# deepreinforce-ai/CUDA-L2

Measured on AMD Instinct MI355X. Metric: HGEMM TFLOP/s, higher is better.
Workload: dtype f16

## Files before the change

cuda-l2_amd/build.py:

```python
from __future__ import annotations

import concurrent.futures as cf
import hashlib
import os
import shutil
import subprocess
import sys
from pathlib import Path

PKG_DIR = Path(__file__).resolve().parent
REPO_DIR = PKG_DIR.parent
CSRC = PKG_DIR / "csrc"
INCLUDE = REPO_DIR / "include"
BUILD = PKG_DIR / "build"
OBJ = BUILD / "obj"
_SUFFIX = os.environ.get("HGEMM_LIB_SUFFIX", "")
LIB_DIR = PKG_DIR / ("lib_" + _SUFFIX if _SUFFIX else "lib")
BIN_DIR = PKG_DIR / "bin"
ROCM = Path(os.environ.get("ROCM_PATH", "/opt/rocm"))
HIPCC = str(ROCM / "bin" / "hipcc")
ARCH = "gfx950"

LIB_SOURCES = [
    "hgemm_inst_g0.hip",
    "hgemm_inst_g1.hip",
    "hgemm_inst_g2.hip",
    "hgemm_inst_g3.hip",
    "hgemm_inst_g4.hip",
    "hgemm_registry.hip",
    "hgemm_plan.hip",
    "hgemm_api.hip",
    "hgemm_baselines.hip",
]

HIP_FLAGS = os.environ.get("HGEMM_EXTRA_HIPFLAGS", "").split() + [f"--offload-arch={ARCH}", "-O3", "-std=c++17", "-fPIC", "-Wall", "-Wno-unused-function",
             "-Wno-unused-result", "-Wno-unused-value", "-DROCBLAS_NO_DEPRECATED_WARNINGS", "-D__HIP_PLATFORM_AMD__"]


def _headers_digest() -> str:
    h = hashlib.sha256()
    for d in (CSRC, INCLUDE):
        for p in sorted(d.rglob("*")):
            if p.suffix in (".hpp", ".h", ".def", ".inc"):
                h.update(p.name.encode())
                h.update(p.read_bytes())
    return h.hexdigest()


def _run(cmd: list[str], verbose: bool) -> None:
    if verbose:
        print(" ".join(cmd), flush=True)
    res = subprocess.run(cmd, capture_output=True, text=True)
    if res.returncode != 0:
        sys.stderr.write(res.stdout + res.stderr)
        raise RuntimeError(f"build step failed ({res.returncode}): {' '.join(cmd)}")
    if verbose and (res.stdout or res.stderr):
        print(res.stdout + res.stderr, flush=True)


def compile_object(src: Path, extra_flags: list[str], hdr_digest: str, verbose: bool = False) -> Path:
    OBJ.mkdir(parents=True, exist_ok=True)
# ... 111 lines not shown
```

cuda-l2_amd/csrc/hgemm_api.hip:

```cpp
#include "hgemm_plan.hpp"
#include "../../include/hgemm_mi355x.h"

#include <algorithm>
#include <atomic>
#include <cmath>
#include <cstdint>
#include <cstdlib>
#include <cstring>
#include <mutex>
#include <vector>

using namespace hgemm_mi355x;

namespace {

thread_local int g_last_hip_error = 0;
#ifdef HGEMM_ABLATION
int g_debug_flags = 0;
#endif
#ifdef HGEMM_TIMELINE
unsigned long long* g_timeline = nullptr;
int g_timeline_slots = 0;
unsigned g_timeline_count = 0;
constexpr int kTimelineWgs = 1024;
// ... 182 lines not shown
        t.tail_first = (int)full; t.tail_tiles = (int)tail; t.splits = S; t.k_chunk = per_t * e.kgran;
        t.items = (int)tail * S;
        g.items = (int)full; set_raster_div(g); set_raster_div(t);
        p.form = FORM_HYBRID; p.slab_bytes = (size_t)t.items * e.bm * e.bn * sizeof(float);
        add(THUNK_ENTRY, g, std::min<long>(full, G), EPI_C16);
        add(THUNK_ENTRY, t, std::min<long>(t.items, G), EPI_SLAB);
        add(THUNK_TAIL_REDUCE, t, 0, EPI_SLAB);
        return p;
      }
    }
  }
  long launch_grid = (e.persistent_wgs > 0) ? std::min<long>(grid, e.persistent_wgs) : grid;
  if (epi == EPI_FUSED && e.persistent_wgs > kCUs && 2L * (e.lds_bytes + 64) > 160L * 1024) launch_grid = std::min<long>(launch_grid, kCUs);
  set_raster_div(g);
  add(THUNK_ENTRY, g, launch_grid, epi);
  if (epi == EPI_SLAB) add(THUNK_SPLITK_REDUCE, g, 0, EPI_SLAB);
  return p;
}

struct AltRow { int M, N, K; const char* cfg; int splits, group_m; };
const AltRow g_alt_rows[] = {
#include "hgemm_tuned_alternates.inc"
    {0, 0, 0, nullptr, 0, 0}};
struct PlanTriple { int cfg, splits, group_m; };
struct InsituChoice { int dev, M, N, K; PlanTriple plan; };
std::mutex g_insitu_mutex;
std::vector<InsituChoice> g_insitu;
std::atomic<unsigned> g_insitu_epoch{1};
std::atomic<int> g_insitu_mode{-1};
constexpr int kInsituReps = 5;
struct InsituMemo { unsigned epoch; int dev, M, N, K; PlanTriple plan; };
thread_local InsituMemo t_insitu_memo[32] = {};

bool insitu_enabled() {
  int mode = g_insitu_mode.load(std::memory_order_relaxed);
  if (mode < 0) {
    const char* e = getenv("HGEMM_MI355X_INSITU");
    int expected = -1;
    g_insitu_mode.compare_exchange_strong(expected, (e && *e && *e != '0') ? 1 : 0);
    mode = g_insitu_mode.load(std::memory_order_relaxed);
  }
  return mode == 1;
}

int insitu_candidates(int M, int N, int K, PlanTriple out[3]) {
  int n = 0;
  PlanTriple p0;
  if (hgemm_mi355x_plan(M, N, K, &p0.cfg, &p0.splits, &p0.group_m) != HGEMM_OK) return 0;
  out[n++] = p0;
  auto add = [&](PlanTriple p) {
    if (n >= 3 || p.cfg < 0 || p.cfg >= g_num_kernels || !k_ok(g_kernel_table[p.cfg], K)) return;
    for (int i = 0; i < n; ++i)
      if (out[i].cfg == p.cfg && out[i].splits == p.splits && out[i].group_m == p.group_m) return;
    out[n++] = p;
  };
  for (const AltRow* r = g_alt_rows; r->cfg; ++r)
    if (r->M == M && r->N == N && r->K == K) add({hgemm_mi355x_config_by_name(r->cfg), r->splits, r->group_m});
  std::call_once(g_tuned_once, build_tuned_index);
  if (p0.cfg >= 0 && !find_tuned(M, N, K) && K % 8 == 0 && (N & 3) == 0) {
    RankedPlan ranked[8];
    int nr = 0, c0, s0, g0;
    if (neighbour_plan(M, N, K, &c0, &s0, &g0, ranked, &nr)) {
      std::sort(ranked, ranked + nr, [](const RankedPlan& a, const RankedPlan& b) { return a.us < b.us; });
      for (int i = 0; i < nr; ++i) add({ranked[i].cfg, ranked[i].splits, ranked[i].group_m});
    }
  }
// ... 259 lines not shown
    return resolve_launch(config_id, splits_arg, group_m, b != nullptr, b_col_major != nullptr, aligned, M, N, K, lda, ldb, ldc, ruled_out);
  };
  LaunchPlan p = resolve();
  float* slabs = nullptr; unsigned* counters = nullptr;
  while (p.status == HGEMM_OK && p.slab_bytes) {
    const int st = ensure_workspace(p.slab_bytes, s, &slabs, &counters);
    if (st == HGEMM_OK) break;
    if (st != HGEMM_ERR_NO_WORKSPACE_INTERNAL && p.form != FORM_HYBRID) return st;
    ruled_out |= 1u << p.form;
    p = resolve();
  }
  if (p.status != HGEMM_OK) return p.status;
  for (int i = 0; i < p.n; ++i) {
    GemmArgs& g = p.d[i].g;
    g.A = (const f16*)a; g.Bt = (const f16*)b_col_major; g.C = (f16*)c;
    if (p.d[i].epi != EPI_C16) {
      g.partial = slabs;
      if (p.counters) g.counters = counters;
    }
    const TimingSlot ts = timing_slot(p.d[i].start, p.d[i].stop);
    switch (p.d[i].thunk) {
      case THUNK_ENTRY: g_kernel_table[config_id].launch(g, p.d[i].grid, s, p.d[i].epi, ts); break;
      case THUNK_SPLITK_REDUCE: launch_splitk_reduce(g.partial, g.C, M, N, ldc, g.splits, s, ts); break;
      case THUNK_TAIL_REDUCE: launch_tail_reduce(g, g_kernel_table[config_id].bm, g_kernel_table[config_id].bn, s, ts); break;
      case THUNK_RAGGED: launch_ragged(g, s, ts); break;
      case THUNK_GENERIC: launch_generic((const f16*)a, (const f16*)b, (f16*)c, M, N, K, lda, N, ldc, s, ts); break;
    }
  }
  hipError_t err = hipGetLastError();
  if (err != hipSuccess) { g_last_hip_error = (int)err; return HGEMM_ERR_HIP; }
  return HGEMM_OK;
}

int hgemm_mi355x_set_insitu(int enable) {
  const int old = insitu_enabled() ? 1 : 0;
  g_insitu_mode.store(enable ? 1 : 0);
  if (!enable) {
    std::lock_guard<std::mutex> lk(g_insitu_mutex);
    g_insitu.clear();
    g_insitu_epoch.fetch_add(1, std::memory_order_release);
  }
  return old;
}

int hgemm_mi355x_insitu_enabled(void) { return insitu_enabled() ? 1 : 0; }

int hgemm_mi355x_insitu_candidates(int M, int N, int K, int config_id[3], int splits[3], int group_m[3]) {
  if (M <= 0 || N <= 0 || K <= 0 || !config_id || !splits || !group_m) return 0;
  PlanTriple c[3];
  const int n = insitu_candidates(M, N, K, c);
  for (int i = 0; i < n; ++i) { config_id[i] = c[i].cfg; splits[i] = c[i].splits; group_m[i] = c[i].group_m; }
  return n;
}

int hgemm_mi355x_insitu_choice(int M, int N, int K, int* config_id, int* splits, int* group_m) {
  PlanTriple p;
  int dev = 0;
  if (hipGetDevice(&dev) != hipSuccess) { (void)hipGetLastError(); dev = 0; }
  if (!config_id || !splits || !group_m || !insitu_lookup(dev, M, N, K, &p)) return 0;
  *config_id = p.cfg; *splits = p.splits; *group_m = p.group_m;
  return 1;
}

int hgemm_mi355x_fp32(const void* a, const void* b, const void* bt, void* c, int M, int N, int K,
                      void* stream) {
  return run(HGEMM_ACC_FP32, a, b, bt, c, M, N, K, stream);
// ... 96 lines not shown
```

cuda-l2_amd/csrc/hgemm_inst.inc:

```
#include "hgemm_launch.hpp"

#define HGEMM_INST_0(...)
#define HGEMM_INST_1(...)
#define HGEMM_INST_2(...)
#define HGEMM_INST_3(...)
#define HGEMM_INST_4(...)
#if HGEMM_INST_GROUP == 0
#undef HGEMM_INST_0
#define HGEMM_INST_0(...) __VA_ARGS__
#elif HGEMM_INST_GROUP == 1
#undef HGEMM_INST_1
#define HGEMM_INST_1(...) __VA_ARGS__
#elif HGEMM_INST_GROUP == 2
#undef HGEMM_INST_2
#define HGEMM_INST_2(...) __VA_ARGS__
#elif HGEMM_INST_GROUP == 3
#undef HGEMM_INST_3
#define HGEMM_INST_3(...) __VA_ARGS__
#elif HGEMM_INST_GROUP == 4
#undef HGEMM_INST_4
#define HGEMM_INST_4(...) __VA_ARGS__
#else
#error "HGEMM_INST_GROUP must be 0..4"
#endif

namespace hgemm_mi355x {
#define HGEMM_THUNK(G, FN, ...) HGEMM_INST_##G(template void FN<__VA_ARGS__>(const GemmArgs&, int, hipStream_t, int, TimingSlot);)
#include "hgemm_thunks.inc"
}
```

cuda-l2_amd/csrc/hgemm_kernel.hpp:

```cpp
#pragma once

#include <hip/hip_runtime.h>
#include <stdint.h>
#include <type_traits>

namespace hgemm_mi355x {

using f16    = _Float16;
using f16x4  = __attribute__((ext_vector_type(4))) _Float16;
using f16x8  = __attribute__((ext_vector_type(8))) _Float16;
using f32x4  = __attribute__((ext_vector_type(4))) float;
using f32x16 = __attribute__((ext_vector_type(16))) float;

constexpr int BK        = 64;
constexpr int ROW_BYTES = BK * 2;
constexpr int NUM_XCD   = 8;

constexpr int ARG_NT_STORE      = 1;
constexpr int ARG_XCD_STAGGER   = 2;
constexpr int ARG_NT_LOADS      = 4;
constexpr int ARG_PHASE_OFFSET  = 8;
constexpr int ARG_WAVE_PRIORITY = 16;
constexpr int ARG_PHASE_OFFSET4 = 32;

// ... 149 lines not shown
}

template <int BYTES>
__device__ __forceinline__ void prefetch_kernargs() {
#if defined(__HIP_DEVICE_COMPILE__)
  const char* ka = (const char*)__builtin_amdgcn_kernarg_segment_ptr();
  unsigned d0, d1, d2, d3;
  if constexpr (BYTES > 192)
    asm volatile("s_load_dword %0, %4, 0x0\n\ts_load_dword %1, %4, 0x40\n\ts_load_dword %2, %4, 0x80\n\ts_load_dword %3, %4, 0xc0\n\ts_waitcnt lgkmcnt(0)"
                 : "=&s"(d0), "=&s"(d1), "=&s"(d2), "=&s"(d3) : "s"(ka));
  else if constexpr (BYTES > 128)
    asm volatile("s_load_dword %0, %3, 0x0\n\ts_load_dword %1, %3, 0x40\n\ts_load_dword %2, %3, 0x80\n\ts_waitcnt lgkmcnt(0)"
                 : "=&s"(d0), "=&s"(d1), "=&s"(d2) : "s"(ka));
  else if constexpr (BYTES > 64)
    asm volatile("s_load_dword %0, %2, 0x0\n\ts_load_dword %1, %2, 0x40\n\ts_waitcnt lgkmcnt(0)" : "=&s"(d0), "=&s"(d1) : "s"(ka));
  else
    asm volatile("s_load_dword %0, %1, 0x0\n\ts_waitcnt lgkmcnt(0)" : "=&s"(d0) : "s"(ka));
  (void)d0; (void)d1; (void)d2; (void)d3;
#endif
}

#ifdef HGEMM_ABLATION
#define HGEMM_DBG(g, bit) (((g).debug & (bit)) != 0)
#else
#define HGEMM_DBG(g, bit) false
#endif

constexpr int EPI_C16    = 0;
constexpr int EPI_SLAB   = 1;
constexpr int EPI_FUSED  = 2;
constexpr int EPI_STREAMK = 3;
constexpr int EPI_KTAIL = 8;
constexpr int EPI_KSTAGGER = 16;

template <int BM_, int BN_, int WM_, int WN_, int MI_, int NBUF_>
struct Cfg {
  static constexpr int BM = BM_, BN = BN_, WM = WM_, WN = WN_, MI = MI_, NBUF = NBUF_;
  static constexpr int NW          = WM * WN;
  static constexpr int THREADS     = NW * 64;
  static constexpr int TM          = BM / WM;
  static constexpr int TN          = BN / WN;
  static constexpr int FM          = TM / MI;
  static constexpr int FN          = TN / MI;
  static constexpr int STAGE_BYTES = (BM + BN) * ROW_BYTES;
  static constexpr int LDS_BYTES   = STAGE_BYTES * NBUF;
  static constexpr int NI_A        = BM / 8;
  static constexpr int NI          = (BM + BN) / 8;
  static constexpr int NJ          = (NI + NW - 1) / NW;
  static_assert(MI == 16 || MI == 32, "MFMA shape");
  static_assert(BM % (WM * MI) == 0 && BN % (WN * MI) == 0, "wave tile must be MFMA-aligned");
  static_assert(BM % 8 == 0 && BN % 8 == 0, "tile rows come in 8-row DMA pieces");
  static_assert(LDS_BYTES <= 160 * 1024, "LDS budget");
  static_assert(NBUF >= 2, "need at least double buffering");
  static_assert(NBUF == 2 || NI % NW == 0, "deep ring needs an even piece split");
};

template <int N>
__device__ __forceinline__ void wait_vmcnt() {
  asm volatile("s_waitcnt vmcnt(%0)" ::"n"(N) : "memory");
}

struct TileCoord {
  int split, m0, n0, k_begin, nk;
  int tile, item;
  float* slab;
  int slab_ld;
// ... 547 lines not shown
```

cuda-l2_amd/csrc/hgemm_kernel_sq.hpp:

```cpp
#pragma once

#include "hgemm_kernel_sp.hpp"

#ifndef HGEMM_SQ_SLACK
#define HGEMM_SQ_SLACK 6
#endif
#ifndef HGEMM_SQ_SLACK32
#define HGEMM_SQ_SLACK32 4
#endif
#ifndef HGEMM_SQ_RS64
#define HGEMM_SQ_RS64 2
#endif
#ifndef HGEMM_SQ_ABL
#define HGEMM_SQ_ABL 0
#endif

namespace hgemm_mi355x {

template <int BM_, int BN_, int WM_, int WN_, int KT_ = 1, int MI_ = 16>
struct CfgSQ : Cfg<BM_, BN_, WM_, WN_, MI_, 2> {
  using Base = Cfg<BM_, BN_, WM_, WN_, MI_, 2>;
  static constexpr int KT  = KT_;
  static constexpr int KS  = (MI_ == 16) ? 1 : 2;
  static constexpr int SL  = KT * KS;
  static constexpr int ACC = (MI_ == 16) ? 4 : 16;
  static constexpr int SUB_BYTES   = Base::STAGE_BYTES;
  static constexpr int STAGE_BYTES = KT * SUB_BYTES;
  static constexpr int LDS_BYTES   = 2 * STAGE_BYTES;
  static constexpr int NFA = Base::FM * SL, NFB = Base::FN * SL;
  static constexpr int T   = Base::FM * Base::FN * SL;
  static constexpr int PA  = Base::NI_A / Base::NW;
  static constexpr int PB  = Base::NJ - PA;
  static constexpr int NJA = KT * PA, NJB = KT * PB;
  static constexpr int RS  = (T >= 64) ? HGEMM_SQ_RS64 : 1;
  static constexpr int SLACK = (MI_ == 32) ? HGEMM_SQ_SLACK32 : (T >= 64) ? HGEMM_SQ_SLACK : (T >= 32 ? 6 : 2);
// ... 125 lines not shown
  constexpr int S = PHASE == 0 ? CFG::P : CFG::Q;
  const uint32_t lds_l = (uint32_t)(uintptr_t)(lds_void_t*)stage_l + (uint32_t)wave * 1024u;
  const uint32_t lds_e = (uint32_t)(uintptr_t)(lds_void_t*)stage_e + (uint32_t)wave * 1024u;
#pragma unroll
  for (int n = 0; n < T; ++n) {
    const int u = n / (FM * FN), i = (n / FN) % FM, j = n % FN;
    if (n == S) {
      __builtin_amdgcn_sched_barrier(0);
      if (!(HGEMM_SQ_ABL & 4)) __builtin_amdgcn_s_waitcnt(kWaitLgkm0);
      if (!(HGEMM_SQ_ABL & 1)) sp_sync();
    }
    sp_mfma_mi<CFG::MI>(i * FN + j, bf[u * FN + j], af[u * FM + i]);
    if (!(HGEMM_SQ_ABL & 16) && n % RS == 0 && n / RS < NLEAD) {
      const int r = n / RS;
      lead[r] = *(const f16x8*)((r / FLEAD ? lead1 : lead0) + (r % FLEAD) * CFG::MI * ROW_BYTES);
    }
    constexpr SqSlots<CFG, PHASE> tab{};
    const int l = (HGEMM_SQ_ABL & 8) ? -1 : tab.late[n], l1 = (HGEMM_SQ_ABL & 8) ? -1 : tab.late[n + 1];
    const int e = (HGEMM_SQ_ABL & 8) ? -1 : tab.early[n], e1 = (HGEMM_SQ_ABL & 8) ? -1 : tab.early[n + 1];
    const int r = (HGEMM_SQ_ABL & 16) ? -1 : tab.trail[n];
    if (l >= 0) { if constexpr (OP_L == 0) sq_piece_load<CFG, 0>(rs_l, voffA, D_L + l, kbyte_l); else sq_piece_load<CFG, 1>(rs_l, voffB, D_L + l, kbyte_l); }
    if (e >= 0) { if constexpr (OP_E == 0) sq_piece_load<CFG, 0>(rs_e, voffA, e, kbyte_e); else sq_piece_load<CFG, 1>(rs_e, voffB, e, kbyte_e); }
    if (r >= 0) trail[r] = *(const f16x8*)((r / FTRAIL ? trail1 : trail0) + (r % FTRAIL) * CFG::MI * ROW_BYTES);
    if (l1 >= 0) sq_piece_m0<CFG, OP_L>(lds_l, D_L + l1, l1 > 0);
    if (e1 >= 0) sq_piece_m0<CFG, OP_E>(lds_e, e1, e1 > 0);
    if (n == S - 2 && !(HGEMM_SQ_ABL & 2)) wait_vmcnt<CFG::NJA + CFG::NJB>();
    if (n == T - 3) {
      __builtin_amdgcn_sched_barrier(0);
      __builtin_amdgcn_s_waitcnt(kWaitLgkm0);
      __builtin_amdgcn_sched_barrier(0);
    }
  }
}
#endif

#define SQ_LOAD_ITEM(OP, ITEM)                                                                                 \
  do {                                                                                                         \
                                \
    if (nxt_item != (ITEM)) {                                                                                  \
      const TileCoord itc = map_logical(g, walk.base + walk.first + (ITEM) * walk.stride, BM, BN);             \
      nxt_item = (ITEM);                                                                                       \
      nxt_m0 = __builtin_amdgcn_readfirstlane(itc.m0); nxt_n0 = __builtin_amdgcn_readfirstlane(itc.n0);        \
      nxt_kb = __builtin_amdgcn_readfirstlane(itc.k_begin * 2);                                                \
             \
      nxt_nk = __builtin_amdgcn_readfirstlane(KTAIL ? sq_k_items(g, itc) / (BK * CFG::KT) : itc.nk / CFG::KT);           \
    }                                                                                                          \
    const uintptr_t addr = (OP) == 0 ? reinterpret_cast<uintptr_t>(g.A + (size_t)nxt_m0 * g.lda)               \
                                     : reinterpret_cast<uintptr_t>(g.Bt + (size_t)nxt_n0 * g.ldb);             \
    const uintptr_t uni = ((uintptr_t)(uint32_t)__builtin_amdgcn_readfirstlane((int)(addr >> 32)) << 32) |     \
                          (uint32_t)__builtin_amdgcn_readfirstlane((int)(uint32_t)addr);                       \
    const unsigned long long rows_ = (OP) == 0 ? (unsigned long long)(g.M - nxt_m0) : (unsigned long long)(g.N - nxt_n0); \
    const unsigned long long rem_ = rows_ * (unsigned long long)((OP) == 0 ? g.lda : g.ldb) * 2ull;            \
    const unsigned range_ = (unsigned)__builtin_amdgcn_readfirstlane((int)(rem_ > 0xFFFFFFFFull ? 0xFFFFFFFFu : (unsigned)rem_)); \
    if ((OP) == 0) rsA = __builtin_amdgcn_make_buffer_rsrc((void*)uni, 0, (int)range_, 0x00020000);            \
    else           rsB = __builtin_amdgcn_make_buffer_rsrc((void*)uni, 0, (int)range_, 0x00020000);            \
                                \
    const int stag_ = STAG ? (int)(((uint32_t)(blockIdx.x & (NUM_XCD - 1)) * (uint32_t)nxt_nk) >> 3) : 0;                   \
    cur[OP].kbyte0 = (uint32_t)nxt_kb; cur[OP].kwrap = nxt_nk - stag_;                                         \
    cur[OP].kbyte = (uint32_t)nxt_kb + (uint32_t)stag_ * (uint32_t)(CFG::KT * ROW_BYTES);                      \
    cur[OP].item = (ITEM); cur[OP].kt = 0; cur[OP].nk = nxt_nk;                                                \
  } while (0)

#define SQ_STEP_CURSOR(OP)                                                                   \
  do {                                                                                       \
    ++cur[OP].kt;                                                                            \
    cur[OP].kbyte += CFG::KT * ROW_BYTES;                                                    \
// ... 7 lines not shown
    } else if (cur[OP].item + 1 < walk.count) {               \
      SQ_LOAD_ITEM(OP, cur[OP].item + 1);                     \
    }                                                         \
  } while (0)

#define SQ_FRAG(STAGE, OPOFF, H, U) ((STAGE) + (CFG::KT == 2 ? (H) * CFG::SUB_BYTES : 0) + (OPOFF) + \
                                     foff[CFG::KT == 2 ? (U) : (H)][CFG::KT == 2 ? 0 : (U) % CFG::KS])
#define SQ_K_STEP(YS, ZS, ADV0, ADV1)                                                                           \
  do {                                                                                                          \
    char* st  = smem + (step & 1) * CFG::STAGE_BYTES;                                                           \
    char* nst = smem + ((step + 1) & 1) * CFG::STAGE_BYTES;                                                     \
    sq_interval<CFG, 0>(fX, fU, fV, SQ_FRAG(st, b_base_off, 1, 0), SQ_FRAG(st, b_base_off, 1, 1),               \
                        ZS, SQ_FRAG(nst, a_base_off, 1, 0), SQ_FRAG(nst, a_base_off, 1, 1), wave, voffA, voffB, \
                        rsA, st, cur[0].kbyte, rsB, st, cur[1].kbyte);                                          \
    ADV0;                                                                                                       \
    sq_interval<CFG, 1>(YS, fV, fX, SQ_FRAG(nst, a_base_off, 0, 0), SQ_FRAG(nst, a_base_off, 0, 1),             \
                        fU, SQ_FRAG(nst, b_base_off, 0, 0), SQ_FRAG(nst, b_base_off, 0, 1), wave, voffA, voffB, \
                        rsB, st, cur[1].kbyte, rsA, nst, cur[0].kbyte);                                         \
    ADV1;                                                                                                       \
    ++step;                                                                                                     \
  } while (0)

__device__ __forceinline__ int sq_k_items(const GemmArgs& g, const TileCoord& tc) {
  return (tc.split + 1 == g.splits ? g.K : tc.k_begin + g.k_chunk) - tc.k_begin;
}

template <class CFG, int EPI_>
__global__ void __launch_bounds__(CFG::THREADS) hgemm_tn_sq_kernel(const GemmArgs g) {
  prefetch_kernargs<sizeof(GemmArgs)>();
#if defined(__HIP_DEVICE_COMPILE__)
  constexpr int EPI = EPI_ & 7;
  constexpr bool KTAIL = (EPI_ & EPI_KTAIL) != 0;
  constexpr bool STAG = (EPI_ & EPI_KSTAGGER) != 0;
  static_assert(!KTAIL || CFG::MI == 16, "the K tail is built from 16x16x32 fragments");
  static_assert(!(KTAIL && STAG), "the kstagger variant takes whole stages only (the host drops the flag when K has a tail)");
  constexpr int BM = CFG::BM, BN = CFG::BN, FM = CFG::FM, FN = CFG::FN, NJ = CFG::NJ, MI = CFG::MI;
  constexpr int NFA = CFG::NFA, NFB = CFG::NFB;
  constexpr int NQ = CFG::ACC / 4;

  constexpr bool STAGED = EPI == SP_EPI_WIDE && CFG::WGS == 1 && sp_staged_ok<CFG>(CFG::LDS_BYTES);
#ifdef HGEMM_TIMELINE
  constexpr int TL_EXTRA = 64;
  constexpr int FLAG_BYTES = 64;
#else
  constexpr int TL_EXTRA = 0;
  constexpr int FLAG_BYTES = (CFG::WGS == 2 && EPI != SP_EPI_FUSED) ? 0 : 64;
#endif
  constexpr int STAGED_BYTES = STAGED ? CFG::NW * SP_STAGED_BYTES_PER_WAVE : 0;
  __shared__ __attribute__((aligned(1024))) char smem[CFG::LDS_BYTES + FLAG_BYTES + STAGED_BYTES + TL_EXTRA];

  const int tid  = threadIdx.x;
  HGEMM_TL_STAMP(smem + CFG::LDS_BYTES, 0, tid);
  HGEMM_TL_REALTIME(smem + CFG::LDS_BYTES, 1, tid);
  const int lane = tid & 63;
  const int wave = __builtin_amdgcn_readfirstlane(tid >> 6);
  const int wave_m = wave / CFG::WN;
  const int wave_n = wave % CFG::WN;

  const ItemWalk walk = persistent_walk(g.items);
  if (walk.count == 0) return;

  if (g.flags & (ARG_PHASE_OFFSET | ARG_PHASE_OFFSET4)) {
    const int j = (int)(blockIdx.x >> 3);
    constexpr int both = ARG_PHASE_OFFSET | ARG_PHASE_OFFSET4;
    const int groups = (g.flags & both) == both ? 8 : (g.flags & ARG_PHASE_OFFSET4) ? 4 : 2, grp = j & (groups - 1);
    if (grp != 0 && walk.count > 1) {
      const int nk0 = g.k_chunk / (BK * CFG::KT);
      const int period = nk0 * 2 * CFG::T * (CFG::MI == 32 ? 32 : 16) + CFG::BM * CFG::BN / 12;
      const int spacing = min(period / groups, CFG::BM * CFG::BN / 6);
#pragma clang loop unroll(disable)
      for (int c = 0; c < spacing * grp; c += 1024) __builtin_amdgcn_s_sleep(16);
    }
  }
  if constexpr (CFG::WGS == 2) {
    if (g.flags & ARG_WAVE_PRIORITY) {
      unsigned hw;
      asm volatile("s_getreg_b32 %0, hwreg(HW_REG_HW_ID)" : "=s"(hw));
      if (hw & 1u) __builtin_amdgcn_s_setprio(2);
    }
  }

// ... 37 lines not shown
    }
    SQ_ADVANCE(0);
    SQ_ADVANCE(1);
  }
  __builtin_amdgcn_sched_barrier(0);
#pragma unroll
  for (; zi < NZ; ++zi) sp_zero_acc(zi);
  HGEMM_TL_STAMP(smem + CFG::LDS_BYTES + 64 + STAGED_BYTES, 1, tid);
  wait_vmcnt<CFG::NJA + CFG::NJB>();
  __builtin_amdgcn_s_barrier();
  HGEMM_TL_STAMP(smem + CFG::LDS_BYTES + 64 + STAGED_BYTES, 2, tid);

  f16x8 fX[NFA], fY[NFA], fZ[NFA], fU[NFB], fV[NFB];
#pragma unroll
  for (int r = 0; r < NFA; ++r) {
    fX[r] = *(const f16x8*)(SQ_FRAG(smem, a_base_off, 0, r / FM) + (r % FM) * MI * ROW_BYTES);
    fY[r] = *(const f16x8*)(SQ_FRAG(smem, a_base_off, 1, r / FM) + (r % FM) * MI * ROW_BYTES);
  }
#pragma unroll
  for (int r = 0; r < NFB; ++r) fU[r] = *(const f16x8*)(SQ_FRAG(smem, b_base_off, 0, r / FN) + (r % FN) * MI * ROW_BYTES);
  __builtin_amdgcn_sched_barrier(0);
  __builtin_amdgcn_s_waitcnt(kWaitLgkm0);
  sp_sync();
#pragma unroll
  for (int p = 0; p < CFG::DA; ++p) sq_issue_piece<CFG, 0>(rsA, voffA, smem, wave, p, cur[0].kbyte);

  int step = 0;
  HGEMM_TL_STAMP(smem + CFG::LDS_BYTES, 2, tid);
#pragma clang loop unroll(disable)
  for (int item = 0; item < walk.count; ++item) {
    const TileCoord tc = map_logical(g, walk.base + walk.first + item * walk.stride, BM, BN);
    const int nk = __builtin_amdgcn_readfirstlane(KTAIL ? sq_k_items(g, tc) / (BK * CFG::KT) : tc.nk / CFG::KT);
    HGEMM_TL_STAMP(smem + CFG::LDS_BYTES, 3, tid);
    int t = 0;
#pragma clang loop unroll(disable)
    for (; t + 5 < nk; t += 2) {
      SQ_K_STEP(fY, fZ, SQ_STEP_CURSOR(0), SQ_STEP_CURSOR(1));
      SQ_K_STEP(fZ, fY, SQ_STEP_CURSOR(0), SQ_STEP_CURSOR(1));
    }
#pragma clang loop unroll(disable)
    for (; t + 1 < nk; t += 2) {
      SQ_K_STEP(fY, fZ, SQ_ADVANCE(0), SQ_ADVANCE(1));
      SQ_K_STEP(fZ, fY, SQ_ADVANCE(0), SQ_ADVANCE(1));
    }
    if (t < nk) {
      sq_settle(fX, fY, fU);
      SQ_K_STEP(fY, fZ, SQ_ADVANCE(0), SQ_ADVANCE(1));
#pragma unroll
      for (int r = 0; r < NFA; ++r) fY[r] = fZ[r];
      sq_settle(fX, fY, fU);
    }
    if constexpr (KTAIL) {
      const int k_items = sq_k_items(g, tc), k_full = nk * (BK * CFG::KT);
      if (k_full < k_items) {
        __builtin_amdgcn_sched_barrier(0);
        direct_k_tail<FM, FN>(g, tc.m0, tc.n0, wave_m * CFG::TM, wave_n * CFG::TN, tc.k_begin + k_full, tc.k_begin + k_items, lane,
                              [](int i, int j, const f16x8& b, const f16x8& a) __attribute__((always_inline)) { sp_mfma(i * FN + j, b, a); });
        __builtin_amdgcn_sched_barrier(0);
      }
    }
    HGEMM_TL_STAMP(smem + CFG::LDS_BYTES, 4, tid);
    sp_mfma_drain();
    const bool rezero = item + 1 < walk.count;
    const __amdgpu_buffer_rsrc_t rsP = fused_rsrc(g);
    const int m_wave = tc.m0 + wave_m * CFG::TM, n_wave = tc.n0 + wave_n * CFG::TN;
    (void)rsP; (void)m_wave; (void)n_wave;
    if constexpr (STAGED) {
      __builtin_amdgcn_sched_barrier(0);
      sp_epilogue_staged<CFG>(g, m_wave, n_wave, rezero, smem + CFG::LDS_BYTES + 64 + wave * SP_STAGED_BYTES_PER_WAVE);
    } else if constexpr (MI == 16) {
#pragma unroll
      for (int i = 0; i < FM; ++i) {
        __builtin_amdgcn_sched_barrier(0);
        f32x4 row[FN];
#pragma unroll
        for (int j = 0; j < FN; ++j) row[j] = sp_read_acc(i * FN + j);
        if (rezero) {
#pragma unroll
          for (int j = 0; j < FN; ++j) sp_zero_acc(i * FN + j);
        }
        if constexpr (EPI == SP_EPI_FUSED) {
#pragma unroll
          for (int j = 0; j < FN; ++j) fused_store(rsP, fused_off<CFG::THREADS>(tc.item, BM * BN, i * FN + j, tid), row[j]);
// ... 134 lines not shown
```

cuda-l2_amd/csrc/hgemm_launch.hpp:

```cpp
#pragma once
#include "hgemm_kernel_rs.hpp"
#include "hgemm_kernel_sq.hpp"
#include "hgemm_kernel_wd.hpp"
#include "hgemm_kernel_lu.hpp"

#include <hip/hip_ext.h>

namespace hgemm_mi355x {

struct LaunchTiming { hipEvent_t start = nullptr, stop = nullptr; };
extern thread_local LaunchTiming t_launch_timing;

struct TimingSlot { hipEvent_t start = nullptr, stop = nullptr; };
inline TimingSlot timing_slot(bool first, bool last) {
  TimingSlot s;
  if (first) { s.start = t_launch_timing.start; t_launch_timing.start = nullptr; }
  if (last) { s.stop = t_launch_timing.stop; t_launch_timing.stop = nullptr; }
  return s;
}

#define HGEMM_LAUNCH(KERNEL, GRID, THREADS, STREAM, SLOT, ...)                                              \
  do {                                                                                                      \
    if ((SLOT).start || (SLOT).stop)                                                                        \
      hipExtLaunchKernelGGL(KERNEL, dim3(GRID), dim3(THREADS), 0, STREAM, (SLOT).start, (SLOT).stop, 0,     \
// ... 10 lines not shown
    HGEMM_LAUNCH((hgemm_tn_kernel<CFG, EPI_FUSED>), grid, CFG::THREADS, stream, ts, g);
  else if (epi == EPI_SLAB)
    HGEMM_LAUNCH((hgemm_tn_kernel<CFG, EPI_SLAB>), grid, CFG::THREADS, stream, ts, g);
  else
    HGEMM_LAUNCH((hgemm_tn_kernel<CFG, EPI_C16>), grid, CFG::THREADS, stream, ts, g);
}

template <class CFG>
void launch_sp(const GemmArgs& g, int grid, hipStream_t stream, int epi, TimingSlot ts) {
  const bool wide = ((g.N & 7) == 0) && ((g.ldc & 7) == 0) && ((reinterpret_cast<uintptr_t>(g.C) & 15) == 0);
  if (epi == EPI_FUSED)
    HGEMM_LAUNCH((hgemm_tn_sp_kernel<CFG, SP_EPI_FUSED>), grid, CFG::THREADS, stream, ts, g);
  else if (epi == EPI_SLAB)
    HGEMM_LAUNCH((hgemm_tn_sp_kernel<CFG, SP_EPI_SLAB>), grid, CFG::THREADS, stream, ts, g);
  else if (wide)
    HGEMM_LAUNCH((hgemm_tn_sp_kernel<CFG, SP_EPI_WIDE>), grid, CFG::THREADS, stream, ts, g);
  else
    HGEMM_LAUNCH((hgemm_tn_sp_kernel<CFG, SP_EPI_NARROW>), grid, CFG::THREADS, stream, ts, g);
}

template <class CFG, int FLAG>
void launch_sq_variant(const GemmArgs& g, int grid, hipStream_t stream, int epi, TimingSlot ts) {
  const bool wide = ((g.N & 7) == 0) && ((g.ldc & 7) == 0) && ((reinterpret_cast<uintptr_t>(g.C) & 15) == 0);
  if (epi == EPI_FUSED)
    HGEMM_LAUNCH((hgemm_tn_sq_kernel<CFG, SP_EPI_FUSED | FLAG>), grid, CFG::THREADS, stream, ts, g);
  else if (epi == EPI_SLAB)
    HGEMM_LAUNCH((hgemm_tn_sq_kernel<CFG, SP_EPI_SLAB | FLAG>), grid, CFG::THREADS, stream, ts, g);
  else if (wide)
    HGEMM_LAUNCH((hgemm_tn_sq_kernel<CFG, SP_EPI_WIDE | FLAG>), grid, CFG::THREADS, stream, ts, g);
  else
    HGEMM_LAUNCH((hgemm_tn_sq_kernel<CFG, SP_EPI_NARROW | FLAG>), grid, CFG::THREADS, stream, ts, g);
}

template <class CFG>
void launch_sq(const GemmArgs& g, int grid, hipStream_t stream, int epi, TimingSlot ts) {
  if constexpr (CFG::MI == 16) {
    if (g.K % (BK * CFG::KT) != 0) return launch_sq_variant<CFG, EPI_KTAIL>(g, grid, stream, epi, ts);
    if (g.flags & ARG_XCD_STAGGER) return launch_sq_variant<CFG, EPI_KSTAGGER>(g, grid, stream, epi, ts);
  }
  launch_sq_variant<CFG, 0>(g, grid, stream, epi, ts);
}

template <class CFG, int FLAG>
void launch_rs_variant(const GemmArgs& g, int grid, hipStream_t stream, int epi, TimingSlot ts) {
  if (epi == EPI_FUSED)
    HGEMM_LAUNCH((hgemm_tn_rs_kernel<CFG, EPI_FUSED | FLAG>), grid, CFG::THREADS, stream, ts, g);
  else if (epi == EPI_SLAB)
    HGEMM_LAUNCH((hgemm_tn_rs_kernel<CFG, EPI_SLAB | FLAG>), grid, CFG::THREADS, stream, ts, g);
  else
    HGEMM_LAUNCH((hgemm_tn_rs_kernel<CFG, EPI_C16 | FLAG>), grid, CFG::THREADS, stream, ts, g);
}

template <class CFG>
void launch_rs(const GemmArgs& g, int grid, hipStream_t stream, int epi, TimingSlot ts) {
  if (epi == EPI_STREAMK)
    HGEMM_LAUNCH((hgemm_tn_rs_sk_kernel<CFG>), grid, CFG::THREADS, stream, ts, g);
  else if (g.K % CFG::BKS != 0)
    launch_rs_variant<CFG, EPI_KTAIL>(g, grid, stream, epi, ts);
  else
    launch_rs_variant<CFG, 0>(g, grid, stream, epi, ts);
}

template <class CFG>
void launch_wd(const GemmArgs& g, int grid, hipStream_t stream, int epi, TimingSlot ts) {
  if (epi == EPI_FUSED)
    HGEMM_LAUNCH((hgemm_tn_wd_kernel<CFG, EPI_FUSED>), grid, CFG::THREADS, stream, ts, g);
  else if (epi == EPI_SLAB)
    HGEMM_LAUNCH((hgemm_tn_wd_kernel<CFG, EPI_SLAB>), grid, CFG::THREADS, stream, ts, g);
// ... 42 lines not shown
```

cuda-l2_amd/csrc/hgemm_thunks.inc:

```
#define HGEMM_CFG(G, BM, BN, WM, WN, MI, NB) HGEMM_THUNK(G, launch_cfg, Cfg<BM, BN, WM, WN, MI, NB>)
#define HGEMM_SP(G, BM, BN, WM, WN, MI) HGEMM_THUNK(G, launch_sp, CfgSP<BM, BN, WM, WN, MI>)
#define HGEMM_SQ(G, BM, BN, WM, WN, KT, MI) HGEMM_THUNK(G, launch_sq, CfgSQ<BM, BN, WM, WN, KT, MI>)
#define HGEMM_RS(G, BM, BN, BKS, LB) HGEMM_THUNK(G, launch_rs, CfgRS<BM, BN, BKS, LB>)
#define HGEMM_WD(G, FM, FN, KW) HGEMM_THUNK(G, launch_wd, CfgWD<FM, FN, KW>)
#include "hgemm_configs.def"
#define HGEMM_LU(BM, BN, WM, WN, NIMG, NB) HGEMM_THUNK(4, launch_lu, CfgLU<BM, BN, WM, WN, NIMG, NB>)
#include "hgemm_configs_lu.def"
#undef HGEMM_THUNK
```

include/hgemm_mi355x.h:

```cpp
#ifndef HGEMM_MI355X_H_
#define HGEMM_MI355X_H_

#include <stddef.h>

#ifdef __cplusplus
extern "C" {
#endif

typedef enum {
  HGEMM_OK = 0,
  HGEMM_ERR_BAD_ARG = -1,
  HGEMM_ERR_TOO_LARGE = -2,
  HGEMM_ERR_HIP = -3,
  HGEMM_ERR_BACKEND = -4,
  HGEMM_ERR_NOT_READY = -5,
  HGEMM_ERR_NO_ALGO = -6,
  HGEMM_ERR_NO_WORKSPACE = -7
} hgemm_status_t;

typedef enum { HGEMM_ACC_FP32 = 0, HGEMM_ACC_FP16 = 1 } hgemm_acc_t;

#define HGEMM_CONFIG_GENERIC (-1)
#define HGEMM_CONFIG_RAGGED  (-2)

#define HGEMM_SPLITK_FUSED 0x10000
#define HGEMM_SPLITK_MASK  0x0ffff
#define HGEMM_PLAN_NT_STORE 0x20000
#define HGEMM_PLAN_STREAMK 0x40000

#define HGEMM_PLAN_RS_XCD_STAGGER 0x80000
#define HGEMM_PLAN_RS_NT_LOADS    0x100000
#define HGEMM_PLAN_XCD_STAGGER HGEMM_PLAN_RS_XCD_STAGGER
#define HGEMM_PLAN_PHASE_OFFSET  0x200000
#define HGEMM_PLAN_WAVE_PRIORITY 0x400000
#define HGEMM_PLAN_PHASE_OFFSET4 0x800000
#define HGEMM_PLAN_PHASE_OFFSET8 (HGEMM_PLAN_PHASE_OFFSET | HGEMM_PLAN_PHASE_OFFSET4)

int hgemm_mi355x_fp32(const void* a, const void* b, const void* b_col_major, void* c,
                      int M, int N, int K, void* stream);
int hgemm_mi355x_fp16(const void* a, const void* b, const void* b_col_major, void* c,
                      int M, int N, int K, void* stream);

int hgemm_mi355x_launch(int config_id, int splits, int group_m,
                        const void* a, const void* b, const void* b_col_major, void* c,
                        int M, int N, int K, int lda, int ldb, int ldc, void* stream);

int hgemm_mi355x_set_insitu(int enable);
int hgemm_mi355x_insitu_enabled(void);
int hgemm_mi355x_insitu_candidates(int M, int N, int K, int config_id[3], int splits[3], int group_m[3]);
int hgemm_mi355x_insitu_choice(int M, int N, int K, int* config_id, int* splits, int* group_m);

int hgemm_mi355x_plan(int M, int N, int K, int* config_id, int* splits, int* group_m);

double hgemm_mi355x_model_us(int config_id, int splits, int M, int N, int K);

int hgemm_mi355x_default_group(int config_id, int M, int N);

int hgemm_mi355x_num_configs(void);
const char* hgemm_mi355x_config_name(int config_id);
int hgemm_mi355x_config_info(int config_id, int out[8]);
int hgemm_mi355x_config_by_name(const char* name);
int hgemm_mi355x_config_k_granularity(int config_id);
int hgemm_mi355x_config_accepts_k(int config_id, int K);
int hgemm_mi355x_config_local_splits(int config_id);
int hgemm_mi355x_config_streamk(int config_id);
int hgemm_mi355x_streamk_runs(int config_id, int M, int N, int K);

int hgemm_mi355x_set_workspace(void* device_ptr, size_t bytes);
int hgemm_mi355x_release_stream_workspace(void* stream);
size_t hgemm_mi355x_workspace_bytes(int M, int N, int splits);
size_t hgemm_mi355x_plan_workspace_bytes(int config_id, int splits, int M, int N, int K);
int hgemm_mi355x_reserve_workspace(int M, int N, int K, void* stream);
int hgemm_mi355x_release_workspaces(void);

const char* hgemm_mi355x_strerror(int status);
int hgemm_mi355x_last_hip_error(void);
const char* hgemm_mi355x_version(void);

int hgemm_rocblas_init(void);
int hgemm_rocblas_destroy(void);
// ... 33 lines not shown
```

Measured before the change: 1483.

## Fold staged C epilogue into the last K step's MFMAs for SQ 256x256

Adds a fold variant of the SQ kernel for the 256x256 config. On each workgroup's last tile, the final K step's MFMAs are interleaved with the staged epilogue's LDS writes, LDS reads and buffer stores, following a compile-time schedule plan. The aim is to hide the epilogue tail behind the last matrix math instead of running it after the accumulators drain. It is enabled by default through an environment switch and adds a new instantiation group, at the cost of extra code complexity and possible register or LDS pressure.

```diff
diff --git a/cuda-l2_amd/build.py b/cuda-l2_amd/build.py
--- a/cuda-l2_amd/build.py
+++ b/cuda-l2_amd/build.py
@@ -27,6 +27,7 @@
     "hgemm_inst_g2.hip",
     "hgemm_inst_g3.hip",
     "hgemm_inst_g4.hip",
+    "hgemm_inst_g5.hip",
     "hgemm_registry.hip",
     "hgemm_plan.hip",
     "hgemm_api.hip",
diff --git a/cuda-l2_amd/csrc/hgemm_api.hip b/cuda-l2_amd/csrc/hgemm_api.hip
--- a/cuda-l2_amd/csrc/hgemm_api.hip
+++ b/cuda-l2_amd/csrc/hgemm_api.hip
@@ -238,6 +238,20 @@
 struct InsituMemo { unsigned epoch; int dev, M, N, K; PlanTriple plan; };
 thread_local InsituMemo t_insitu_memo[32] = {};
 
+std::atomic<int> g_sq_fold_mode{-1};
+}
+bool hgemm_mi355x::sq_fold_enabled() {
+  int mode = g_sq_fold_mode.load(std::memory_order_relaxed);
+  if (mode < 0) {
+    const char* e = getenv("HGEMM_MI355X_SQ_FOLD");
+    int expected = -1;
+    g_sq_fold_mode.compare_exchange_strong(expected, (e && *e == '0') ? 0 : 1);
+    mode = g_sq_fold_mode.load(std::memory_order_relaxed);
+  }
+  return mode == 1;
+}
+namespace {
+
 bool insitu_enabled() {
   int mode = g_insitu_mode.load(std::memory_order_relaxed);
   if (mode < 0) {
@@ -563,6 +577,12 @@
   return HGEMM_OK;
 }
 
+int hgemm_mi355x_set_sq_fold(int enable) {
+  const int old = sq_fold_enabled() ? 1 : 0;
+  g_sq_fold_mode.store(enable ? 1 : 0);
+  return old;
+}
+
 int hgemm_mi355x_set_insitu(int enable) {
   const int old = insitu_enabled() ? 1 : 0;
   g_insitu_mode.store(enable ? 1 : 0);
diff --git a/cuda-l2_amd/csrc/hgemm_inst.inc b/cuda-l2_amd/csrc/hgemm_inst.inc
--- a/cuda-l2_amd/csrc/hgemm_inst.inc
+++ b/cuda-l2_amd/csrc/hgemm_inst.inc
@@ -5,6 +5,7 @@
 #define HGEMM_INST_2(...)
 #define HGEMM_INST_3(...)
 #define HGEMM_INST_4(...)
+#define HGEMM_INST_5(...)
 #if HGEMM_INST_GROUP == 0
 #undef HGEMM_INST_0
 #define HGEMM_INST_0(...) __VA_ARGS__
@@ -20,8 +21,11 @@
 #elif HGEMM_INST_GROUP == 4
 #undef HGEMM_INST_4
 #define HGEMM_INST_4(...) __VA_ARGS__
+#elif HGEMM_INST_GROUP == 5
+#undef HGEMM_INST_5
+#define HGEMM_INST_5(...) __VA_ARGS__
 #else
-#error "HGEMM_INST_GROUP must be 0..4"
+#error "HGEMM_INST_GROUP must be 0..5"
 #endif
 
 namespace hgemm_mi355x {
diff --git a/cuda-l2_amd/csrc/hgemm_inst_g5.hip b/cuda-l2_amd/csrc/hgemm_inst_g5.hip
--- /dev/null
+++ b/cuda-l2_amd/csrc/hgemm_inst_g5.hip
@@ -0,0 +1,2 @@
+#define HGEMM_INST_GROUP 5
+#include "hgemm_inst.inc"
diff --git a/cuda-l2_amd/csrc/hgemm_kernel.hpp b/cuda-l2_amd/csrc/hgemm_kernel.hpp
--- a/cuda-l2_amd/csrc/hgemm_kernel.hpp
+++ b/cuda-l2_amd/csrc/hgemm_kernel.hpp
@@ -205,6 +205,7 @@
 constexpr int EPI_STREAMK = 3;
 constexpr int EPI_KTAIL = 8;
 constexpr int EPI_KSTAGGER = 16;
+constexpr int EPI_FOLD = 32;
 
 template <int BM_, int BN_, int WM_, int WN_, int MI_, int NBUF_>
 struct Cfg {
diff --git a/cuda-l2_amd/csrc/hgemm_kernel_sq.hpp b/cuda-l2_amd/csrc/hgemm_kernel_sq.hpp
--- a/cuda-l2_amd/csrc/hgemm_kernel_sq.hpp
+++ b/cuda-l2_amd/csrc/hgemm_kernel_sq.hpp
@@ -1,6 +1,9 @@
 #pragma once
 
 #include "hgemm_kernel_sp.hpp"
+#include "hgemm_sq_fold_plan.hpp"
+
+#include <utility>
 
 #ifndef HGEMM_SQ_SLACK
 #define HGEMM_SQ_SLACK 6
@@ -192,6 +195,97 @@
     }
   }
 }
+template <class F, int... N>
+__device__ __forceinline__ void sq_static_for(F&& f, std::integer_sequence<int, N...>) { (f(std::integral_constant<int, N>{}), ...); }
+
+template <class CFG>
+__device__ __forceinline__ void sq_fold_step(const GemmArgs& g, int m_wave, int n_wave, char* stage,
+                                             const f16x8 (&x)[CFG::NFA], const f16x8 (&y)[CFG::NFA], const f16x8 (&u)[CFG::NFB], f16x8 (&v)[CFG::NFB],
+                                             const char* vsrc, char* tl_slots, int tid) {
+  constexpr int FM = CFG::FM, FN = CFG::FN;
+  using PL = SqFoldPlan<FM, FN>;
+  constexpr int NG = PL::NG;
+  using h2 = __attribute__((ext_vector_type(2))) _Float16;
+  using u4 = __attribute__((ext_vector_type(4))) unsigned;
+  (void)tl_slots; (void)tid;
+#pragma unroll
+  for (int j = 0; j < FN; ++j) v[j] = *(const f16x8*)(vsrc + j * CFG::MI * ROW_BYTES);
+  __builtin_amdgcn_sched_barrier(0);
+  __builtin_amdgcn_s_waitcnt(kWaitLgkm0);
+  __builtin_amdgcn_sched_barrier(0);
+#pragma unroll
+  for (int r = 0; r < CFG::NFA; ++r) asm volatile("" ::"v"(x[r]), "v"(y[r]));
+#pragma unroll
+  for (int r = 0; r < CFG::NFB; ++r) asm volatile("" ::"v"(u[r]), "v"(v[r]));
+  asm volatile("s_nop 1");
+  unsigned waddr[4], raddr = 0, voff[NG], row8 = 0;
+  __amdgpu_buffer_rsrc_t rsC;
+  const bool nt = (g.flags & ARG_NT_STORE) != 0;
+  u4 rb[2][2];
+  auto setup = [&]() __attribute__((always_inline)) {
+    int lane;
+    asm volatile("v_mbcnt_lo_u32_b32 %0, -1, 0\n\tv_mbcnt_hi_u32_b32 %0, -1, %0" : "=v"(lane));
+    const unsigned lds0 = (unsigned)(uintptr_t)(__attribute__((address_space(3))) char*)stage;
+    const int wrow = lane & 15, wq = lane >> 4;
+#pragma unroll
+    for (int jj = 0; jj < 4; ++jj) waddr[jj] = lds0 + wrow * 128 + (((jj * 2 + (wq >> 1)) ^ (wrow & 7)) << 4) + (wq & 1) * 8;
+    const int rrow = lane >> 3, rch = lane & 7;
+    raddr = lds0 + rrow * 128 + ((rch ^ (rrow & 7)) << 4);
+    const uintptr_t caddr = reinterpret_cast<uintptr_t>(g.C + (size_t)m_wave * g.ldc + n_wave);
+    const uintptr_t cuni = ((uintptr_t)(uint32_t)__builtin_amdgcn_readfirstlane((int)(caddr >> 32)) << 32) |
+                           (uint32_t)__builtin_amdgcn_readfirstlane((int)(uint32_t)caddr);
+    const long long rem = ((long long)(g.M - m_wave) * g.ldc - n_wave) * 2;
+    const unsigned range = __builtin_amdgcn_readfirstlane((int)(rem <= 0 ? 0 : rem > 0x7FFFFFFFLL ? 0x7FFFFFFF : rem));
+    rsC = __builtin_amdgcn_make_buffer_rsrc((void*)cuni, 0, (int)range, 0x00020000);
+#pragma unroll
+    for (int gg = 0; gg < NG; ++gg)
+      voff[gg] = (n_wave + gg * 64 + rch * 8 < g.N) ? (unsigned)(rrow * g.ldc + gg * 64 + rch * 8) * 2u : 0x80000000u;
+    row8 = (unsigned)g.ldc * 16u;
+  };
+  auto op = [&](auto qc) __attribute__((always_inline)) {
+    constexpr int q = decltype(qc)::value;
+    constexpr PL plan{};
+    constexpr int kind = plan.kind[q], k = plan.group[q], jj = plan.tile[q], i = k / NG, gg = k % NG, b = k & 1;
+    if constexpr (kind == PL::W) {
+      const f32x4 a = sp_read_acc(i * FN + gg * 4 + jj);
+      const h2 lo = {(f16)a[0], (f16)a[1]}, hi = {(f16)a[2], (f16)a[3]};
+      const unsigned long long pk = (unsigned long long)__builtin_bit_cast(unsigned, lo) | ((unsigned long long)__builtin_bit_cast(unsigned, hi) << 32);
+      if constexpr (b) asm volatile("ds_write_b64 %0, %1 offset:2048" ::"v"(waddr[jj]), "v"(pk) : "memory");
+      else             asm volatile("ds_write_b64 %0, %1" ::"v"(waddr[jj]), "v"(pk) : "memory");
+    } else if constexpr (kind == PL::R) {
+      if constexpr (b) {
+        asm volatile("ds_read_b128 %0, %1 offset:2048" : "=v"(rb[1][0]) : "v"(raddr) : "memory");
+        asm volatile("ds_read_b128 %0, %1 offset:3072" : "=v"(rb[1][1]) : "v"(raddr) : "memory");
+      } else {
+        asm volatile("ds_read_b128 %0, %1" : "=v"(rb[0][0]) : "v"(raddr) : "memory");
+        asm volatile("ds_read_b128 %0, %1 offset:1024" : "=v"(rb[0][1]) : "v"(raddr) : "memory");
+      }
+    } else {
+      asm volatile("s_waitcnt lgkmcnt(0)" : "+v"(rb[b][0]), "+v"(rb[b][1])::"memory");
+      if (!HGEMM_DBG(g, 2)) {
+#pragma unroll
+        for (int h = 0; h < 2; ++h) {
+          if (nt) __builtin_amdgcn_raw_buffer_store_b128(rb[b][h], rsC, voff[gg], (unsigned)(i * 2 + h) * row8, 2);
+          else    __builtin_amdgcn_raw_buffer_store_b128(rb[b][h], rsC, voff[gg], (unsigned)(i * 2 + h) * row8, 0);
+        }
+      }
+    }
+  };
+  sq_static_for([&](auto nc) __attribute__((always_inline)) {
+    constexpr int n = decltype(nc)::value;
+    constexpr PL plan{};
+    constexpr int i = PL::mfma_row(n), s = PL::mfma_slice(n), j = PL::mfma_col(n);
+    if constexpr (s == 0) sp_mfma(i * FN + j, u[j], x[i]); else sp_mfma(i * FN + j, v[j], y[i]);
+    if constexpr (n == 0) setup();
+    if constexpr (plan.at[n] >= 0) op(std::integral_constant<int, plan.at[n]>{});
+  }, std::make_integer_sequence<int, PL::T2>{});
+  HGEMM_TL_STAMP(tl_slots, 4, tid);
+  sp_mfma_drain();
+  __builtin_amdgcn_sched_barrier(0);
+  constexpr int n_hidden = PL{}.n_hidden;
+  sq_static_for([&](auto qc) __attribute__((always_inline)) { op(std::integral_constant<int, n_hidden + decltype(qc)::value>{}); },
+                std::make_integer_sequence<int, PL::NOPS - n_hidden>{});
+}
 #endif
 
 #define SQ_LOAD_ITEM(OP, ITEM)                                                                                 \
@@ -265,6 +359,7 @@
   constexpr int EPI = EPI_ & 7;
   constexpr bool KTAIL = (EPI_ & EPI_KTAIL) != 0;
   constexpr bool STAG = (EPI_ & EPI_KSTAGGER) != 0;
+  constexpr bool FOLD = (EPI_ & EPI_FOLD) != 0;
   static_assert(!KTAIL || CFG::MI == 16, "the K tail is built from 16x16x32 fragments");
   static_assert(!(KTAIL && STAG), "the kstagger variant takes whole stages only (the host drops the flag when K has a tail)");
   constexpr int BM = CFG::BM, BN = CFG::BN, FM = CFG::FM, FN = CFG::FN, NJ = CFG::NJ, MI = CFG::MI;
@@ -280,6 +375,8 @@
   constexpr int FLAG_BYTES = (CFG::WGS == 2 && EPI != SP_EPI_FUSED) ? 0 : 64;
 #endif
   constexpr int STAGED_BYTES = STAGED ? CFG::NW * SP_STAGED_BYTES_PER_WAVE : 0;
+  static_assert(!FOLD || (STAGED && !KTAIL && !STAG && CFG::MI == 16 && CFG::KT == 1),
+                "the fold variant: staged epilogue, whole stages of K = 64, 16x16x32 fragments, no K stagger");
   __shared__ __attribute__((aligned(1024))) char smem[CFG::LDS_BYTES + FLAG_BYTES + STAGED_BYTES + TL_EXTRA];
 
   const int tid  = threadIdx.x;
@@ -383,23 +480,34 @@
     const TileCoord tc = map_logical(g, walk.base + walk.first + item * walk.stride, BM, BN);
     const int nk = __builtin_amdgcn_readfirstlane(KTAIL ? sq_k_items(g, tc) / (BK * CFG::KT) : tc.nk / CFG::KT);
     HGEMM_TL_STAMP(smem + CFG::LDS_BYTES, 3, tid);
+    const bool fold_item = FOLD && item + 1 == walk.count;
+    const int nkl = fold_item ? nk - 1 : nk;
     int t = 0;
 #pragma clang loop unroll(disable)
-    for (; t + 5 < nk; t += 2) {
+    for (; t + 5 < nkl; t += 2) {
       SQ_K_STEP(fY, fZ, SQ_STEP_CURSOR(0), SQ_STEP_CURSOR(1));
       SQ_K_STEP(fZ, fY, SQ_STEP_CURSOR(0), SQ_STEP_CURSOR(1));
     }
 #pragma clang loop unroll(disable)
-    for (; t + 1 < nk; t += 2) {
+    for (; t + 1 < nkl; t += 2) {
       SQ_K_STEP(fY, fZ, SQ_ADVANCE(0), SQ_ADVANCE(1));
       SQ_K_STEP(fZ, fY, SQ_ADVANCE(0), SQ_ADVANCE(1));
     }
-    if (t < nk) {
+    if (t < nkl) {
       sq_settle(fX, fY, fU);
       SQ_K_STEP(fY, fZ, SQ_ADVANCE(0), SQ_ADVANCE(1));
 #pragma unroll
       for (int r = 0; r < NFA; ++r) fY[r] = fZ[r];
       sq_settle(fX, fY, fU);
+    }
+    if constexpr (FOLD) {
+      if (fold_item) {
+        sq_fold_step<CFG>(g, tc.m0 + wave_m * CFG::TM, tc.n0 + wave_n * CFG::TN, smem + CFG::LDS_BYTES + 64 + wave * SP_STAGED_BYTES_PER_WAVE,
+                          fX, fY, fU, fV, SQ_FRAG(smem + (step & 1) * CFG::STAGE_BYTES, b_base_off, 1, 0), smem + CFG::LDS_BYTES, tid);
+        ++step;
+        HGEMM_TL_STAMP(smem + CFG::LDS_BYTES, 5, tid);
+        break;
+      }
     }
     if constexpr (KTAIL) {
       const int k_items = sq_k_items(g, tc), k_full = nk * (BK * CFG::KT);
diff --git a/cuda-l2_amd/csrc/hgemm_launch.hpp b/cuda-l2_amd/csrc/hgemm_launch.hpp
--- a/cuda-l2_amd/csrc/hgemm_launch.hpp
+++ b/cuda-l2_amd/csrc/hgemm_launch.hpp
@@ -66,8 +66,24 @@
     HGEMM_LAUNCH((hgemm_tn_sq_kernel<CFG, SP_EPI_NARROW | FLAG>), grid, CFG::THREADS, stream, ts, g);
 }
 
+bool sq_fold_enabled();
+template <class CFG> inline constexpr bool sq_has_fold = false;
+template <> inline constexpr bool sq_has_fold<CfgSQ<256, 256, 2, 2, 1, 16>> = true;
+template <class CFG>
+void launch_sq_fold(const GemmArgs& g, int grid, hipStream_t stream, int, TimingSlot ts) {
+  HGEMM_LAUNCH((hgemm_tn_sq_kernel<CFG, SP_EPI_WIDE | EPI_FOLD>), grid, CFG::THREADS, stream, ts, g);
+}
+#if !defined(HGEMM_INST_GROUP) || HGEMM_INST_GROUP != 5
+extern template void launch_sq_fold<CfgSQ<256, 256, 2, 2, 1, 16>>(const GemmArgs&, int, hipStream_t, int, TimingSlot);
+#endif
+
 template <class CFG>
 void launch_sq(const GemmArgs& g, int grid, hipStream_t stream, int epi, TimingSlot ts) {
+  if constexpr (sq_has_fold<CFG>) {
+    const bool wide = ((g.N & 7) == 0) && ((g.ldc & 7) == 0) && ((reinterpret_cast<uintptr_t>(g.C) & 15) == 0);
+    if (epi == EPI_C16 && wide && g.K % (BK * CFG::KT) == 0 && !(g.flags & ARG_XCD_STAGGER) && sq_fold_enabled())
+      return launch_sq_fold<CFG>(g, grid, stream, epi, ts);
+  }
   if constexpr (CFG::MI == 16) {
     if (g.K % (BK * CFG::KT) != 0) return launch_sq_variant<CFG, EPI_KTAIL>(g, grid, stream, epi, ts);
     if (g.flags & ARG_XCD_STAGGER) return launch_sq_variant<CFG, EPI_KSTAGGER>(g, grid, stream, epi, ts);
diff --git a/cuda-l2_amd/csrc/hgemm_sq_fold_plan.hpp b/cuda-l2_amd/csrc/hgemm_sq_fold_plan.hpp
--- /dev/null
+++ b/cuda-l2_amd/csrc/hgemm_sq_fold_plan.hpp
@@ -0,0 +1,42 @@
+#pragma once
+
+namespace hgemm_mi355x {
+
+template <int FM, int FN>
+struct SqFoldPlan {
+  static_assert(FN % 4 == 0, "the staged epilogue works on groups of four tiles");
+  static constexpr int NG = FN / 4, G = FM * NG, T2 = 2 * FM * FN, NOPS = 6 * G;
+  static constexpr int DRAIN = 3;
+  enum : int { W = 0, R = 1, S = 2 };
+  static constexpr int mfma_row(int n) { return n / (2 * FN); }
+  static constexpr int mfma_slice(int n) { return (n / FN) % 2; }
+  static constexpr int mfma_col(int n) { return n % FN; }
+  static constexpr int last_mfma_of_row(int i) { return 2 * FN * (i + 1) - 1; }
+
+  short kind[NOPS], group[NOPS], tile[NOPS];
+  short gap[NOPS];
+  short at[T2];
+  int n_hidden;
+
+  constexpr SqFoldPlan() : kind(), group(), tile(), gap(), at(), n_hidden(0) {
+    int p = 0;
+    for (int jj = 0; jj < 4; ++jj) { kind[p] = W; group[p] = 0; tile[p] = (short)jj; ++p; }
+    for (int k = 0; k < G; ++k) {
+      kind[p] = R; group[p] = (short)k; tile[p] = 0; ++p;
+      if (k + 1 < G)
+        for (int jj = 0; jj < 4; ++jj) { kind[p] = W; group[p] = (short)(k + 1); tile[p] = (short)jj; ++p; }
+      kind[p] = S; group[p] = (short)k; tile[p] = 0; ++p;
+    }
+    for (int n = 0; n < T2; ++n) at[n] = -1;
+    int prev = 0;
+    for (int q = 0; q < NOPS; ++q) {
+      const int earliest = kind[q] == W ? last_mfma_of_row(group[q] / NG) + DRAIN : 0;
+      const int x = prev + 1 > earliest ? prev + 1 : earliest;
+      gap[q] = (short)x;
+      if (x < T2) { at[x] = (short)q; n_hidden = q + 1; }
+      prev = x;
+    }
+  }
+};
+
+}
diff --git a/cuda-l2_amd/csrc/hgemm_thunks.inc b/cuda-l2_amd/csrc/hgemm_thunks.inc
--- a/cuda-l2_amd/csrc/hgemm_thunks.inc
+++ b/cuda-l2_amd/csrc/hgemm_thunks.inc
@@ -6,4 +6,5 @@
 #include "hgemm_configs.def"
 #define HGEMM_LU(BM, BN, WM, WN, NIMG, NB) HGEMM_THUNK(4, launch_lu, CfgLU<BM, BN, WM, WN, NIMG, NB>)
 #include "hgemm_configs_lu.def"
+HGEMM_THUNK(5, launch_sq_fold, CfgSQ<256, 256, 2, 2, 1, 16>)
 #undef HGEMM_THUNK
diff --git a/include/hgemm_mi355x.h b/include/hgemm_mi355x.h
--- a/include/hgemm_mi355x.h
+++ b/include/hgemm_mi355x.h
@@ -46,6 +46,7 @@
                         int M, int N, int K, int lda, int ldb, int ldc, void* stream);
 
 int hgemm_mi355x_set_insitu(int enable);
+int hgemm_mi355x_set_sq_fold(int enable);
 int hgemm_mi355x_insitu_enabled(void);
 int hgemm_mi355x_insitu_candidates(int M, int N, int K, int config_id[3], int splits[3], int group_m[3]);
 int hgemm_mi355x_insitu_choice(int M, int N, int K, int* config_id, int* splits, int* group_m);
```

After: 1493 (median of 6 runs). No clear change (+0.7%).
